# huggingface/tokenizers

Hardware: NVIDIA H100
Metric: encode_batch input throughput (higher is better)
Workload: dtype u8

## Files before the change

### tokenizers_b200/csrc/engine.cu

```cuda
#include <cuda_runtime.h>
#include <stdarg.h>
#include <stdio.h>
#include <stdlib.h>
#include <string.h>

#include <algorithm>
#include <atomic>
#include <condition_variable>
#include <memory>
#include <mutex>
#include <string>
#include <vector>

#include "../../include/b2t.h"
#include "added_kernels.cuh"
#include "dense_kernels.cuh"
#include "host_tables.h"
#include "long_kernels.cuh"
#include "model_kernels.cuh"
#include "norm_kernels.cuh"
#include "prefix_kernels.cuh"
#include "pretok_kernels.cuh"

using namespace b2t;
// ... 269 lines not shown
    long long v = atoll(cb);
    if (v >= 1024 && v < (1ll << 31)) e->chunk_bytes = (size_t)v;
  }
  int rc = B2T_OK;
  if ((rc = upload(e->d_cls, ht.cls_packed)) || (rc = upload(e->d_byte_to_id, ht.byte_to_id)) || (rc = upload(e->d_merge, ht.merge_tbl)) ||
      (rc = upload(e->d_word, ht.word_tbl)) || (rc = upload(e->d_pool, ht.word_pool)) || (rc = upload(e->d_edge, ht.edge_tbl)) ||
      (rc = upload(e->d_tok2, ht.tok2_bits)) || (rc = upload(e->d_tri, ht.tri_bits)))
    return rc;
  if (cfg->bert_normalizer & B2T_NORM_BERT) {
    NormHost nh;
    build_bert_norm((cfg->bert_normalizer & B2T_NORM_CLEAN_TEXT) != 0, (cfg->bert_normalizer & B2T_NORM_CHINESE_CHARS) != 0,
                    (cfg->bert_normalizer & B2T_NORM_STRIP_ACCENTS) != 0, (cfg->bert_normalizer & B2T_NORM_LOWERCASE) != 0, &nh);
    if (!nh.ok) return fail(B2T_ERR_UNSUPPORTED, "BertNormalizer table: an image exceeds three bytes per input byte");
    if ((rc = upload(e->d_nt_blk, nh.blk)) || (rc = upload(e->d_nt_ent, nh.ent)) || (rc = upload(e->d_nt_pool, nh.pool)) || (rc = upload(e->d_nt_ascii, nh.ascii)))
      return rc;
    e->nt.blk = e->d_nt_blk.as<uint16_t>(); e->nt.ent = e->d_nt_ent.as<uint32_t>(); e->nt.pool = e->d_nt_pool.as<uint8_t>(); e->nt.ascii = e->d_nt_ascii.as<uint8_t>();
    e->norm_on = 1;
  }
  memset(&e->dt, 0, sizeof(e->dt));
  e->dt.byte_to_id = e->d_byte_to_id.as<uint32_t>();
  e->dt.merge_tbl = e->d_merge.as<uint4>();
  e->dt.merge_mask = ht.merge_tbl.empty() ? 0 : (uint32_t)ht.merge_tbl.size() - 1;
  e->dt.word_tbl = e->d_word.as<uint4>();
  e->dt.word_mask = ht.word_tbl.empty() ? 0 : (uint32_t)ht.word_tbl.size() - 1;
  e->dt.word_pool = e->d_pool.as<uint8_t>();
  e->dt.ignore_merges = cfg->ignore_merges ? 1 : 0;
  e->dt.monotone = ht.monotone ? 1 : 0;
  e->dt.tok2_bits = e->d_tok2.as<uint32_t>(); e->dt.tri_bits = e->d_tri.as<uint32_t>();
  e->monotone = e->dt.monotone;
  e->dt.edge_tbl = e->d_edge.as<uint4>();
  e->dt.edge_mask = ht.edge_tbl.empty() ? 0 : (uint32_t)ht.edge_tbl.size() - 1;
  e->dt.unk_id = ht.unk_id;
  e->dt.max_chars = ht.max_chars;
  cudaFuncSetAttribute(model_tile_kernel<MODEL_BPE>, cudaFuncAttributePreferredSharedMemoryCarveout, 86);
  cudaFuncSetAttribute(model_tile_kernel<MODEL_WORDPIECE>, cudaFuncAttributePreferredSharedMemoryCarveout, 86);
  if (cfg->model == B2T_MODEL_BPE) {
    if ((rc = upload(e->d_trim_vocab, vocab_trim_counts(cfg->n_vocab, cfg->vocab_bytes, cfg->vocab_off, cfg->vocab_ids)))) return rc;
    e->trim_ready = 1;
  }
  cudaError_t se = cudaStreamCreateWithFlags(&e->own_stream, cudaStreamNonBlocking);
  if (se != cudaSuccess) return fail(B2T_ERR_CUDA, "cudaStreamCreate failed: %s", cudaGetErrorString(se));
  *out = e.release();
  return B2T_OK;
}

extern "C" void b2t_engine_destroy(b2t_engine* e) {
  if (!e) return;
  cudaSetDevice(e->device);
  cudaDeviceSynchronize();
  delete e;
}

struct ctl_block {
  uint32_t max_row;
  uint32_t err;
  unsigned long long total;
  LongCtl lc;
  uint32_t added_used;
  uint32_t max_all;
  unsigned long long rows;
  uint32_t stride_m;
  uint32_t pad;
};

static int ensure_long_pool(Workspace& ws, unsigned long long bytes) {
  if (bytes <= ws.pool_cap) return B2T_OK;
  unsigned long long cap = bytes + bytes / 4 + 4096;
  int rc;
// ... 358 lines not shown
    case PT_GPT2: launch_pretok<PT_GPT2>(e, d_bytes, n, ws, st, added); break;
    case PT_LLAMA3: launch_pretok<PT_LLAMA3>(e, d_bytes, n, ws, st, added); break;
    case PT_WHITESPACE: launch_pretok<PT_WHITESPACE>(e, d_bytes, n, ws, st, added); break;
    case PT_BERT: launch_pretok<PT_BERT>(e, d_bytes, n, ws, st, added); break;
    default: launch_pretok<PT_NOREGEX>(e, d_bytes, n, ws, st, added); break;
  }
  rec(e, st, "pretok_scan"); e->last_launches++;
  const int64_t n_scan_blocks = (n_pages + SCAN_BLOCK - 1) / SCAN_BLOCK;
  page_scan_block_kernel<<<(unsigned)n_scan_blocks, SCAN_BLOCK, 0, st>>>(ws.page_sum.as<uint64_t>(), ws.page_carry.as<uint64_t>(),
                                                                      ws.block_sum.as<uint64_t>(), n_pages);
  page_scan_top_kernel<<<1, SCAN_BLOCK, 0, st>>>(ws.block_sum.as<uint64_t>(), ws.block_carry.as<uint64_t>(), n_scan_blocks);
  rec(e, st, "page_scan"); e->last_launches += 2;
  return B2T_OK;
}

static void long_pretokens(b2t_engine* e, Workspace& ws, const Batch& b, cudaStream_t st) {
  const uint8_t* d_bytes = b.bytes; const int64_t n = b.n;
  const int64_t n_pages = n / PAGE + 1;
  ctl_block* ctl = ws.ctl.as<ctl_block>();
  LongPool pool;
  pool.id = ws.lp_id.as<uint32_t>(); pool.val = ws.lp_val.as<uint64_t>(); pool.len = ws.lp_len.as<uint32_t>(); pool.plen = ws.lp_plen.as<uint32_t>();
  pool.aux = ws.lp_aux.as<uint32_t>(); pool.out = ws.lp_out.as<uint4>(); pool.cap = ws.pool_cap;
  long_find_kernel<0><<<(unsigned)((n_pages + 7) / 8), 256, 0, st>>>(ws.start_bits.as<uint32_t>(), nullptr, nullptr, n, n_pages, &ctl->lc,
                                                                    ws.long_desc1.as<LongDesc>(), nullptr, 0ull);
  soft_cut_kernel<<<(unsigned)(e->sm_count * 4), 256, 0, st>>>(d_bytes, &ctl->lc, ws.long_desc1.as<LongDesc>(), ws.soft_bits.as<uint32_t>(),
                                                             ws.page_soft.as<uint8_t>(), e->dt);
  long_find_kernel<1><<<(unsigned)((n_pages + 7) / 8), 256, 0, st>>>(ws.start_bits.as<uint32_t>(), ws.soft_bits.as<uint32_t>(), ws.page_soft.as<uint8_t>(),
                                                                    n, n_pages, &ctl->lc, ws.long_desc.as<LongDesc>(), ws.page_long.as<int32_t>(), ws.pool_cap);
  rec(e, st, "long_find"); e->last_launches += 3;
  bpe_long_kernel<<<(unsigned)(e->sm_count * 2), LONG_THREADS, 0, st>>>(d_bytes, &ctl->lc, ws.long_desc.as<LongDesc>(), pool, e->dt, e->monotone);
  rec(e, st, "bpe_long"); e->last_launches++;
}

static void model_and_count(b2t_engine* e, Workspace& ws, const Batch& b, uint32_t flags, bool added, cudaStream_t st) {
  const int64_t n_pages = b.n / PAGE + 1;
  ModelParams P;
  P.bytes = b.bytes; P.n = b.n;
  P.start_bits = ws.start_bits.as<uint32_t>(); P.drop_bits = ws.drop_bits.as<uint32_t>(); P.doc_bits = ws.doc_bits.as<uint32_t>();
  P.soft_bits = ws.soft_bits.as<uint32_t>(); P.page_soft = ws.page_soft.as<uint8_t>();
  P.page_carry = ws.page_carry.as<uint64_t>(); P.block_carry = ws.block_carry.as<uint64_t>(); P.page_first_doc = ws.page_first_doc.as<uint32_t>();
  P.doc_off = b.doc_off; P.n_docs = b.n_docs;
  P.flags = ((flags & B2T_WANT_OFFSETS) ? F_OFFSETS : 0u) | ((flags & B2T_WANT_WORD_IDS) ? F_WORD_IDS : 0u) |
            (((flags & B2T_OFFSETS_BYTES) || ws.norm_active) ? F_BYTE_OFFSETS : 0u);
  P.ids = ws.tmp_ids.as<uint32_t>(); P.offsets = ws.tmp_offsets.as<uint32_t>(); P.word_ids = ws.tmp_word_ids.as<uint32_t>();
  P.row_ptr = ws.row_ptr_local.as<uint64_t>();
  P.tile_count = ws.tile_count.as<uint32_t>(); P.tile_first = ws.tile_first.as<uint32_t>();
  ctl_block* ctl = ws.ctl.as<ctl_block>();
  P.err_flag = &ctl->err;
  P.n_tiles = n_pages;
  P.page_long = ws.page_long.as<int32_t>(); P.long_desc = ws.long_desc.as<LongDesc>(); P.long_out = ws.lp_out.as<uint4>();
  P.wcache = ws.wcache.as<uint4>(); P.wcache_mask = WCACHE_SLOTS - 1; P.wcache_on = e->wcache_on;
  P.prefix_bits = b.prefix_bits;
  P.added_bits = added ? ws.added_bits.as<uint32_t>() : nullptr; P.added_head = ws.added_head.as<uint32_t>(); P.added_pool = ws.added_pool.as<uint2>();
  P.flag_added = (flags & B2T_FLAG_ADDED_IDS) ? 1u : 0u;
  P.t = e->dt;
  if (e->model == B2T_MODEL_BPE) model_tile_kernel<MODEL_BPE><<<(unsigned)n_pages, MODEL_THREADS, 0, st>>>(P);
  else model_tile_kernel<MODEL_WORDPIECE><<<(unsigned)n_pages, MODEL_THREADS, 0, st>>>(P);
  rec(e, st, e->model == B2T_MODEL_BPE ? "bpe_tile" : "wordpiece_tile"); e->last_launches++;
  const int64_t n_tblk = (n_pages + TSCAN - 1) / TSCAN;
  tile_scan_block_kernel<<<(unsigned)n_tblk, TSCAN, 0, st>>>(ws.tile_count.as<uint32_t>(), ws.tile_lexcl.as<unsigned long long>(),
                                                           ws.tile_bsum.as<unsigned long long>(), n_pages);
  tile_scan_top_kernel<<<1, TSCAN, 0, st>>>(ws.tile_bsum.as<unsigned long long>(), n_tblk, &ctl->total);
  e->last_launches += 2;
}

static int finish_tail(b2t_engine* e, Workspace& ws, cudaStream_t st) {
  const DenseReq* dq = ws.req.dq;
  const bool finish = ws.req.until == RUN_RESULT;
  const uint32_t n_docs = ws.batch.n_docs;
  int rc;
  if (finish && (rc = finish_device(e, ws, ws.ids.as<uint32_t>(), ws.offsets.as<uint32_t>(), ws.word_ids.as<uint32_t>(), ws.row_ptr.as<uint64_t>(), 0ull, st)))
    return rc;
  rec(e, st, "scan_compact");
  if (dq && finish) {
    ctl_block* ctl = ws.ctl.as<ctl_block>();
    const uint32_t n_rows = n_docs / dq->docs_per_row;
    const PairDenseSpec& P = dq->P;
    if (n_rows && dq->pairs())
      pair_len_max_kernel<<<(n_rows + 255) / 256, 256, 0, st>>>(ws.row_ptr.as<uint64_t>(), n_rows, P.budget, P.strategy, P.n_pre + P.n_mid + P.n_post,
                                                              &ctl->max_row, &ctl->err);
    else if (n_rows)
      row_len_max_kernel<<<(n_rows + 255) / 256, 256, 0, st>>>(ws.row_ptr.as<uint64_t>(), n_rows, dq->S.keep_max, dq->S.n_pre + dq->S.n_post, &ctl->max_row);
    e->last_launches++;
    if (dq->overflow) {
      const uint32_t budget = dq->pairs() ? P.budget : dq->S.keep_max, n_special = dq->pairs() ? P.n_pre + P.n_mid + P.n_post : dq->S.n_pre + dq->S.n_post;
      const int64_t n_blk = ((int64_t)n_rows + TSCAN - 1) / TSCAN;
      if ((rc = ws.row_count.ensure((size_t)n_rows * 4 + 16)) || (rc = ws.row_lexcl.ensure((size_t)n_rows * 8 + 16)) ||
          (rc = ws.row_bsum.ensure((size_t)n_blk * 8 + 16)))
        return rc;
      if (n_rows) {
        dense_count_kernel<<<(n_rows + 255) / 256, 256, 0, st>>>(ws.row_ptr.as<uint64_t>(), n_rows, dq->pairs() ? 1u : 0u, budget, dq->pairs() ? P.strategy : 0u, dq->stride,
                                                               n_special, ws.row_count.as<uint32_t>(), &ctl->max_all, &ctl->err, &ctl->stride_m);
        tile_scan_block_kernel<<<(unsigned)n_blk, TSCAN, 0, st>>>(ws.row_count.as<uint32_t>(), ws.row_lexcl.as<unsigned long long>(),
                                                                 ws.row_bsum.as<unsigned long long>(), n_rows);
        tile_scan_top_kernel<<<1, TSCAN, 0, st>>>(ws.row_bsum.as<unsigned long long>(), n_blk, &ctl->rows);
        e->last_launches += 3;
      }
      rec(e, st, "dense_count");
    } else {
      if (!dq->batch_longest && (rc = launch_dense(e, ws, n_rows, n_rows, *dq, st))) return rc;
      rec(e, st, dq->pairs() ? "dense_pair_rows" : "dense_rows");
    }
  }
  CU(cudaMemcpyAsync(ws.h_ctl.p, ws.ctl.p, sizeof(ctl_block), cudaMemcpyDeviceToHost, st));
  return B2T_OK;
}

static int run_device_pipeline(b2t_engine* e, Workspace& ws, cudaStream_t st) {
  const Request& q = ws.req;
  if (q.n + (int64_t)q.n_docs >= (1ll << 31)) return fail(B2T_ERR_TOO_LARGE, "batch of %lld bytes exceeds the per-call limit of 2^31-1; split it", (long long)q.n);
  Batch& b = ws.batch;
  b = Batch{q.bytes, q.n, q.doc_off, q.n_docs, nullptr};
  e->last_launches = 0;
  const bool model_pass = q.until != RUN_PRETOK;
  int rc;
  if ((rc = repack_prefix(e, ws, b, st)) || (rc = normalize(e, ws, b, q.flags, st)) || (rc = size_buffers(e, ws, b, q.flags, model_pass, st)))
    return rc;
  const bool added = e->has_added && !(q.flags & B2T_NO_ADDED_TOKENS) && b.n > 0 && b.n_docs > 0;
  if ((rc = scan(e, ws, b, added, st))) return rc;
  if (model_pass) {
    if (e->model == B2T_MODEL_BPE) long_pretokens(e, ws, b, st);
    model_and_count(e, ws, b, q.flags, added, st);
    if ((rc = finish_tail(e, ws, st))) return rc;
  }
  CU(cudaGetLastError());
  return B2T_OK;
}

static int trim_ambiguous() {
  return fail(B2T_ERR_UNSUPPORTED, "offset trimming: an added token with both lstrip and rstrip absorbed whitespace, and its offsets do not tell "
              "on which side; trim_offsets is not available for this batch");
}

static int meta_check(b2t_engine* e, Workspace& ws, const DenseReq& dq, cudaStream_t st) {
  if (!dq.trim || !e->has_added || !e->added_both) return B2T_OK;
  ctl_block* h = ws.h_ctl.as<ctl_block>();
  CU(cudaMemcpyAsync(&h->err, &ws.ctl.as<ctl_block>()->err, 4, cudaMemcpyDeviceToHost, st));
  CU(cudaStreamSynchronize(st));
  if (h->err & ERR_INTERNAL) return fail(B2T_ERR_CUDA, "internal error: a marked added-token id without an added token");
  return (h->err & ERR_TRIM_AMBIGUOUS) ? trim_ambiguous() : B2T_OK;
}

static int check_run(b2t_engine* e, Workspace& ws, cudaStream_t st, bool* reran = nullptr) {
  for (int attempt = 0;; ++attempt) {
    const ctl_block* c = ws.h_ctl.as<ctl_block>();
    if (c->err & ERR_ADDED_UNSUPPORTED)
      return fail(B2T_ERR_UNSUPPORTED, "added-token extraction: a span over %d bytes, more spans than one per 16 input bytes, or overlapping spans; "
                  "pass B2T_NO_ADDED_TOKENS and split on the host", ADDED_MAX_SPAN);
    if ((c->err | c->lc.err) & ERR_INTERNAL) return fail(B2T_ERR_CUDA, "internal error: long pre-token / added-token bookkeeping mismatch");
    if (!(c->lc.err & ERR_POOL_OVERFLOW)) {
      if (c->err & ERR_TRUNCATION) return fail(B2T_ERR_TRUNCATION, "Truncation error: Sequence to truncate too short to respect the provided max_length");
      if (c->err & ERR_STRIDE)
        return fail(B2T_ERR_TRUNCATION, "`stride` must be strictly less than `max_len=%u` (note that `max_len` may be shorter than the max length of the "
                    "original model, as it subtracts the number of special characters", c->stride_m);
      if (c->err & ERR_TRIM_AMBIGUOUS) return trim_ambiguous();
      return B2T_OK;
// ... 575 lines not shown
```

### tokenizers_b200/csrc/model_kernels.cuh

```cuda
#pragma once
#include <cuda_runtime.h>
#include <stdint.h>
#include <type_traits>
#include "b2t_tables.h"
#include "added_kernels.cuh"
#include "long_kernels.cuh"
#include "pretok_logic.cuh"

namespace b2t {

constexpr int TILE = PAGE;
constexpr int MODEL_THREADS = 256;
constexpr int THREAD_PATH_MAX = 32;
enum { MODEL_BPE = 0, MODEL_WORDPIECE = 1 };
enum { F_OFFSETS = 1u, F_WORD_IDS = 2u, F_BYTE_OFFSETS = 4u };
constexpr int MAX_LONG_PER_PAGE = TILE / (LONG_PRETOK_MIN + 1) + 1;

struct ModelParams {
  const uint8_t* bytes; int64_t n;
  const uint32_t* start_bits; const uint32_t* drop_bits; const uint32_t* doc_bits;
  const uint32_t* soft_bits; const uint8_t* page_soft;
  const uint64_t* page_carry; const uint64_t* block_carry; const uint32_t* page_first_doc;
  const uint64_t* doc_off; uint32_t n_docs;
  uint32_t flags;
  uint32_t* ids; uint32_t* offsets; uint32_t* word_ids; uint64_t* row_ptr;
  uint32_t* tile_count; uint32_t* tile_first; uint32_t* err_flag;
  int64_t n_tiles;
  const int32_t* page_long; const LongDesc* long_desc; const uint4* long_out;
  uint4* wcache; uint32_t wcache_mask; int wcache_on;
  const uint32_t* prefix_bits;
  const uint32_t* added_bits; const uint32_t* added_head; const uint2* added_pool; uint32_t flag_added;
  DeviceTables t;
};

__device__ __forceinline__ uint64_t merge_lookup(const DeviceTables& t, uint32_t a, uint32_t b) {
  const uint32_t hf = pair_hash(a, b);
  uint32_t h = hf & t.merge_mask;
  while (true) {
    uint4 e = __ldg(t.merge_tbl + h);
    if (e.x == a && e.y == b) return ((uint64_t)e.z << 32) | e.w;
    if (e.x == EMPTY_KEY) return NO_MERGE;
    h = (h + 1) & t.merge_mask;
  }
}

__device__ __forceinline__ int warp_prefix_words(const uint32_t* bits, uint16_t* pref, int nw, int lane) {
  int c0 = 0, c1 = 0, c2 = 0;
  int i = lane * 3;
  if (i < nw) c0 = __popc(bits[i]);
  if (i + 1 < nw) c1 = __popc(bits[i + 1]);
  if (i + 2 < nw) c2 = __popc(bits[i + 2]);
  int tot = c0 + c1 + c2, inc = tot;
#pragma unroll
  for (int s = 1; s < 32; s <<= 1) {
    int o = __shfl_up_sync(0xFFFFFFFFu, inc, s);
    if (lane >= s) inc += o;
  }
  int ex = inc - tot;
  if (i < nw) pref[i] = (uint16_t)ex;
  if (i + 1 < nw) pref[i + 1] = (uint16_t)(ex + c0);
  if (i + 2 < nw) pref[i + 2] = (uint16_t)(ex + c0 + c1);
  return __shfl_sync(0xFFFFFFFFu, inc, 31);
}

__device__ __forceinline__ uint32_t mask_le(int b) { return b >= 31 ? 0xFFFFFFFFu : ((2u << b) - 1u); }

constexpr int TOK_ID_BITS = 20;
__device__ __forceinline__ uint32_t tok_pack(uint32_t id, int len) { return id | ((uint32_t)len << TOK_ID_BITS); }
__device__ __forceinline__ int tok_len(uint32_t x) { return (int)(x >> TOK_ID_BITS); }
__device__ __forceinline__ uint32_t tok_id(uint32_t x) { return x & ((1u << TOK_ID_BITS) - 1u); }


constexpr int WC_MAX_BYTES = 24, WC_MAX_TOK = 6, WC_PROBES = 4;
constexpr int P4_SPLIT_BYTES = 16;
constexpr int P4_SHORT_G = 8;
#define B2T_WC_READY (1ull << 63)
#define B2T_WC_BUSY (1ull << 62)
#define B2T_WC_FP ((1ull << 62) - 1ull)

struct WordKey {
  uint32_t k[6];
  uint32_t slot;
  unsigned long long fp;
};

__device__ __forceinline__ void wc_make_key(const uint8_t* s_byte, int s, int len, WordKey& key) {
  const uint32_t* w = reinterpret_cast<const uint32_t*>(s_byte) + (s >> 2);
  const uint32_t sh = (uint32_t)(s & 3) * 8u;
  uint32_t a0 = w[0], a1 = w[1], a2 = w[2], a3 = w[3], a4 = w[4], a5 = w[5], a6 = w[6];
  uint32_t k[6] = {__funnelshift_r(a0, a1, sh), __funnelshift_r(a1, a2, sh), __funnelshift_r(a2, a3, sh),
                   __funnelshift_r(a3, a4, sh), __funnelshift_r(a4, a5, sh), __funnelshift_r(a5, a6, sh)};
#pragma unroll
  for (int i = 0; i < 6; ++i) {
    const int v = min(len - 4 * i, 4);
    const uint32_t m = __funnelshift_rc(0xFFFFFFFFu, 0u, (uint32_t)(32 - 8 * v));
    key.k[i] = k[i] & m;
  }
  uint32_t a = key.k[0] ^ (key.k[2] * 0x9E3779B1u) ^ (key.k[4] * 0x85EBCA77u);
// ... 155 lines not shown
          const int q = bp + tok_len(s_tok[bp]);
          s_tok[bp] = tok_pack(nid, nx - bp); s_tok[q] = 0u;
        }
        if (p > bp && p < nx) rk[j] = 0xFFFFFFFFu;
      }
    }
    __syncwarp();
    if (have) {
      const uint32_t newid = tok_id(s_tok[bp]);
#pragma unroll
      for (int j = 0; j < J; ++j) {
        const int p = s + gl + G * j;
        if (p == bp) {
          rk[j] = 0xFFFFFFFFu;
          if (nx < e) { const uint64_t v = merge_lookup(t, newid, tok_id(s_tok[nx])); rk[j] = (uint32_t)(v >> 32); ni[j] = (uint32_t)v; }
        } else if (p == pv) {
          const uint64_t v = merge_lookup(t, tok_id(s_tok[pv]), newid); rk[j] = (uint32_t)(v >> 32); ni[j] = (uint32_t)v;
        }
      }
    }
  }
}


__device__ __forceinline__ int bit_rank_incl(const uint16_t* pref, const uint32_t* bits, int x) {
  return (int)pref[x >> 5] + __popc(bits[x >> 5] & mask_le(x & 31));
}
__device__ __forceinline__ bool bit_at(const uint32_t* bits, int x) { return (bits[x >> 5] >> (x & 31)) & 1u; }

template <int HALO_>
struct PageCommon {
  static constexpr int HALO = HALO_, SPAN = TILE + HALO, NW = SPAN / 32, TW = TILE / 32;
  static_assert(NW <= 96 && SPAN % 16 == 0, "warp_prefix_words handles <= 96 words; tok is 16-byte aligned");
  uint8_t byte[SPAN];
  uint32_t tok[SPAN];
  long long span_doc_start;
  uint32_t startb[NW + 1], keptb[NW + 1], leadb[NW + 1], tokb[NW + 1], dsb[TW + 1], addedb[TW + 1];
  uint16_t apref[NW + 1], spref[NW + 1], lpref[NW + 1], tpref[NW + 1];
  int16_t dlast[TW + 1];
  uint16_t pt[TILE + 2], list[SPAN];
  int tile, npt, elast, is_long, ntok, nmiss;
};
struct BpePage : PageCommon<256> {
  uint16_t mq[TILE / THREAD_PATH_MAX + 2], lk[MAX_LONG_PER_PAGE + 1];
  int nmiss_hi, nmq, anysoft, nl, lcum[MAX_LONG_PER_PAGE + 2];
  unsigned long long loff[MAX_LONG_PER_PAGE + 1];
};
struct WpPage : PageCommon<416> {
  long long long_end;
  int next, long_chars;
};
template <int MODEL> using PageState = std::conditional_t<MODEL == MODEL_BPE, BpePage, WpPage>;

__device__ __forceinline__ int long_tokens_before(const BpePage& sh, int x) {
  int c = 0;
  for (int a = 0; a < sh.nl; ++a) if ((int)sh.pt[sh.lk[a]] < x) c = sh.lcum[a + 1];
  return c;
}
__device__ __forceinline__ int long_tokens_before(const WpPage&, int) { return 0; }

__device__ __forceinline__ bool is_piece(const BpePage& sh, int64_t base, int64_t n, int s, int e) {
  if (!sh.anysoft) return false;
  const bool real_e = base + e >= n || (e < BpePage::SPAN && bit_at(sh.keptb, e));
  return !(bit_at(sh.keptb, s) && real_e);
}

template <class S>
__device__ __forceinline__ bool added_at(const ModelParams& P, const S& sh, int s) { return P.added_bits != nullptr && bit_at(sh.addedb, s); }
__device__ __forceinline__ uint32_t added_id(const ModelParams& P, int64_t t, int s) {
  for (uint32_t i = __ldg(P.added_head + t); i != ADDED_NIL;) {
    const uint2 v = __ldg(P.added_pool + i);
    if ((int)(v.x & (uint32_t)(PAGE - 1)) == s) return v.x >> 11;
    i = v.y;
  }
  atomicOr(P.err_flag, ERR_INTERNAL);
  return 0u;
}

__device__ __forceinline__ void warp_enqueue(uint16_t* q, int* len, bool take, int k, bool back) {
  const int lane = threadIdx.x & 31;
  const unsigned m = __ballot_sync(0xFFFFFFFFu, take);
  int b = 0;
  if (lane == 0 && m) b = atomicAdd(len, __popc(m));
  b = __shfl_sync(0xFFFFFFFFu, b, 0) + __popc(m & ((1u << lane) - 1u));
  if (take) q[back ? -b : b] = (uint16_t)k;
}

__device__ __forceinline__ bool whole_word_gate(const ModelParams& P, const uint8_t* s_byte, uint32_t* s_tok, int s, int e, bool ask, int leader) {
  if (!P.t.ignore_merges) return false;
  const int whole = ask && vocab_whole_word(P.t, s_byte, s, e - s, s_tok) ? 1 : 0;
  return __shfl_sync(0xFFFFFFFFu, whole, leader) != 0;
}

__device__ __forceinline__ int64_t char_boundary(const ModelParams& P, int64_t g, int step) {
  while ((step < 0 ? g > 0 : g < P.n) && (__ldg(P.bytes + g) & 0xC0u) == 0x80u) g += step;
  return g;
}

struct DocOrigin { int64_t ds; int cb; uint32_t wid; };
template <class S>
__device__ __forceinline__ DocOrigin doc_origin(const ModelParams& P, const S& sh, int64_t base, int x) {
  const int xx = x < TILE ? x : TILE - 1;
  const uint32_t m = sh.dsb[xx >> 5] & mask_le(xx & 31);
  const int D = m ? (xx & ~31) + 31 - __clz((int)m) : (int)sh.dlast[xx >> 5];
  int2 carry = make_int2(0, 0);
  if (D < 0) {
    const uint64_t c = __ldg(P.page_carry + sh.tile);
    const uint64_t bc = (c >> 31) & 1ull ? 0ull : __ldg(P.block_carry + (sh.tile >> 10));
    carry = make_int2((int)(((uint32_t)c & 0x7FFFFFFFu) + (uint32_t)bc), (int)((uint32_t)(c >> 32) + (uint32_t)(bc >> 32)));
  }
  DocOrigin o;
  o.ds = D >= 0 ? base + D : sh.span_doc_start;
  o.cb = D >= 0 ? bit_rank_incl(sh.lpref, sh.leadb, D) - 1 : -carry.x;
  const int wb = D >= 0 ? bit_rank_incl(sh.spref, sh.keptb, D) - (int)bit_at(sh.keptb, D) : -carry.y;
  o.wid = (uint32_t)(bit_rank_incl(sh.spref, sh.keptb, x) - 1 - wb);
  return o;
}

__device__ __forceinline__ void place_token(const ModelParams& P, const DocOrigin& o, unsigned long long out,
                                            int c0, int c1, int64_t g0, int64_t g1) {
  if (P.flags & F_OFFSETS) {
    const bool byte_off = P.flags & F_BYTE_OFFSETS;
    uint32_t o0, o1;
    if (!byte_off) {
      o0 = (uint32_t)(c0 - o.cb); o1 = (uint32_t)(c1 - o.cb);
    } else {
      o0 = (uint32_t)(char_boundary(P, g0, -1) - o.ds); o1 = (uint32_t)(char_boundary(P, g1, 1) - o.ds);
    }
    if (P.prefix_bits && ((__ldg(P.prefix_bits + (o.ds >> 5)) >> (o.ds & 31)) & 1u)) {
      if (o1 == 1u && byte_off) o1 = (uint32_t)(char_boundary(P, o.ds + 2, 1) - o.ds);
      o0 = o0 ? o0 - 1u : 0u;
      o1 = o1 > 2u ? o1 - 1u : 1u;
    }
    reinterpret_cast<uint2*>(P.offsets)[out] = make_uint2(o0, o1);
  }
  if (P.flags & F_WORD_IDS) P.word_ids[out] = o.wid;
}

template <class S>
__device__ __forceinline__ void emit_token(const ModelParams& P, const S& sh, int64_t base, unsigned long long out,
                                           uint32_t id, int ts, int c1, int64_t g1) {
  P.ids[out] = (P.flag_added && ts < TILE && added_at(P, sh, ts)) ? (id | 0x80000000u) : id;
  place_token(P, doc_origin(P, sh, base, ts), out, bit_rank_incl(sh.lpref, sh.leadb, ts) - 1, c1, base + ts, g1);
}

struct PageSpan { int first, eproc, pproc; bool is_long, long_kept; };
template <int MODEL, class S>
__device__ __forceinline__ PageSpan page_span(const S& sh) {
  const int Pn = sh.npt;
  PageSpan r;
  r.is_long = sh.is_long && Pn > 0;
  const bool wp_long = MODEL == MODEL_WORDPIECE && r.is_long;
  r.first = Pn ? (int)sh.pt[0] : sh.elast;
  r.eproc = Pn ? (wp_long ? (int)sh.pt[Pn - 1] : sh.elast) : 0;
  r.pproc = wp_long ? Pn - 1 : Pn;
  r.long_kept = wp_long && bit_at(sh.keptb, sh.pt[Pn - 1]);
  return r;
}

template <int MODEL, class S>
__device__ __forceinline__ void stage_page(const ModelParams& P, S& sh, int64_t t, int64_t base) {
  constexpr int SPAN = S::SPAN, NW = S::NW, TW = S::TW;
  const int tid = threadIdx.x, lane = tid & 31, warp = tid >> 5;
  const int64_t n = P.n, n_chunks = n / CHUNK + 1;
  for (int i = tid; i < SPAN / 16; i += MODEL_THREADS) {
    int64_t g = base + (int64_t)i * 16;
    uint4 v = make_uint4(0, 0, 0, 0);
    if (g + 16 <= n) v = __ldg(reinterpret_cast<const uint4*>(P.bytes + g));
    else if (g < n) {
      uint32_t w[4] = {0, 0, 0, 0};
      for (int k = 0; k < 16 && g + k < n; ++k) w[k >> 2] |= (uint32_t)__ldg(P.bytes + g + k) << (8 * (k & 3));
      v = make_uint4(w[0], w[1], w[2], w[3]);
    }
    reinterpret_cast<uint4*>(sh.byte)[i] = v;
  }
  for (int w = tid; w <= NW; w += MODEL_THREADS) {
// ... 55 lines not shown
          while (e < 0) {
            int64_t w = gw + lane;
            uint32_t b = (w < n_chunks) ? __ldg(P.start_bits + w) : 0u;
            uint32_t any = __ballot_sync(0xFFFFFFFFu, b != 0u);
            if (any) {
              int l = __ffs((int)any) - 1;
              uint32_t bb = __shfl_sync(0xFFFFFFFFu, b, l);
              e = (gw + l) * 32 + (__ffs((int)bb) - 1);
            } else if (gw + 32 >= n_chunks) e = n;
            gw += 32;
          }
          if (lane == 0) sh.long_end = e < n ? e : n;
        }
      }
    } else if (found > lim) found = (int)lim;
    if (lane == 0) { sh.elast = found; sh.is_long = is_long; }
  } else if (warp == 4) {
    uint32_t b0 = sh.dsb[2 * lane], b1 = sh.dsb[2 * lane + 1];
    int last0 = b0 ? (2 * lane) * 32 + 31 - __clz((int)b0) : -1;
    int last1 = b1 ? (2 * lane + 1) * 32 + 31 - __clz((int)b1) : -1;
    int mx = max(last0, last1), inc = mx;
#pragma unroll
    for (int s = 1; s < 32; s <<= 1) {
      int o = __shfl_up_sync(0xFFFFFFFFu, inc, s);
      if (lane >= s) inc = max(inc, o);
    }
    int before = __shfl_up_sync(0xFFFFFFFFu, inc, 1);
    if (lane == 0) before = -1;
    sh.dlast[2 * lane] = (int16_t)before; sh.dlast[2 * lane + 1] = (int16_t)max(before, last0);
    if (lane == 31) sh.dlast[TW] = (int16_t)inc;
  } else if (warp == 5 && lane == 0) {
    uint32_t fd = __ldg(P.page_first_doc + t);
    sh.span_doc_start = fd > 0 ? (long long)__ldg(P.doc_off + fd - 1) : 0;
  }
  __syncthreads();
  if (tid < S::TW) {
    uint32_t bits = sh.startb[tid];
    int idx = sh.apref[tid];
    while (bits) { sh.pt[idx++] = (uint16_t)(tid * 32 + __ffs((int)bits) - 1); bits &= bits - 1u; }
  }
  if (tid == 0) sh.pt[sh.npt] = (uint16_t)sh.elast;
}

__device__ __forceinline__ void collect_long_pretokens(const ModelParams& P, BpePage& sh, int64_t t, int64_t base) {
  const int tid = threadIdx.x, Pn = sh.npt;
  int any_long = 0;
  for (int k = tid; k < Pn; k += MODEL_THREADS)
    if ((int)sh.pt[k + 1] - (int)sh.pt[k] > LONG_PRETOK_MIN) { int i = atomicAdd(&sh.nl, 1); if (i < MAX_LONG_PER_PAGE) sh.lk[i] = (uint16_t)k; any_long = 1; }
  if (!__syncthreads_or(any_long)) return;
  if (tid == 0) {
    int nl = sh.nl;
    if (nl > MAX_LONG_PER_PAGE) { nl = MAX_LONG_PER_PAGE; atomicOr(P.err_flag, ERR_INTERNAL); }
    for (int a = 1; a < nl; ++a) { uint16_t v = sh.lk[a]; int b = a - 1; while (b >= 0 && sh.lk[b] > v) { sh.lk[b + 1] = sh.lk[b]; --b; } sh.lk[b + 1] = v; }
    const int32_t slot0 = nl ? __ldg(P.page_long + t) : 0;
    if (nl && slot0 < 0) { atomicOr(P.err_flag, ERR_INTERNAL); nl = 0; }
    int cum = 0;
    for (int a = 0; a < nl; ++a) {
      const LongDesc d = P.long_desc[slot0 + a];
      if (d.start != base + sh.pt[sh.lk[a]]) atomicOr(P.err_flag, ERR_INTERNAL);
      sh.lcum[a] = cum; sh.loff[a] = d.pool_off;
      cum += (d.pool_off == ~0ull) ? 0 : (int)d.ntok;
    }
    sh.lcum[nl] = cum;
    sh.nl = nl;
  }
  __syncthreads();
  for (int a = 0; a < sh.nl; ++a) {
    const int ls = sh.pt[sh.lk[a]], le = min((int)sh.pt[sh.lk[a] + 1], BpePage::SPAN);
    for (int pos = ls + tid; pos < le; pos += MODEL_THREADS) sh.tok[pos] = 0u;
  }
  __syncthreads();
}
// ... 87 lines not shown
        }
        if (best_end < 0) { bad = true; break; }
        sh.tok[start] = tok_pack(best_id, best_end - start);
        start = best_end;
      }
    }
    if (bad) {
      for (int p = s; p < e; ++p) sh.tok[p] = 0u;
      sh.tok[s] = tok_pack(P.t.unk_id, len);
    }
    wc_publish(P, sh.byte, sh.tok, s, e, false);
  }
  if (sp.is_long) {
    const int64_t ls = base + sh.pt[sh.npt - 1], le = sh.long_end;
    int cnt = 0;
    for (int64_t p = ls + tid; p < le; p += MODEL_THREADS) cnt += ((__ldg(P.bytes + p) & 0xC0u) != 0x80u);
#pragma unroll
    for (int sft = 16; sft >= 1; sft >>= 1) cnt += __shfl_xor_sync(0xFFFFFFFFu, cnt, sft);
    if (lane == 0) atomicAdd(&sh.long_chars, cnt);
  }
}

template <int MODEL, class S>
__device__ __forceinline__ void count_tokens(const ModelParams& P, S& sh, int64_t t, int64_t base) {
  const int tid = threadIdx.x, lane = tid & 31;
  const PageSpan sp = page_span<MODEL>(sh);
  for (int row = tid >> 5; row < S::NW; row += MODEL_THREADS / 32) {
    const int pos = row * 32 + lane;
    const uint32_t tb = __ballot_sync(0xFFFFFFFFu, pos >= sp.first && pos < sp.eproc && tok_len(sh.tok[pos]) != 0);
    if (lane == 0) sh.tokb[row] = tb;
  }
  __syncthreads();
  if (tid < 32) {
    const int tot = warp_prefix_words(sh.tokb, sh.tpref, S::NW, lane);
    if (lane == 0) sh.ntok = tot;
  }
  __syncthreads();
  for (int row = tid >> 5; row < S::NW; row += MODEL_THREADS / 32) {
    const uint32_t tb = sh.tokb[row];
    if ((tb >> lane) & 1u) sh.list[sh.tpref[row] + __popc(tb & ((1u << lane) - 1u))] = (uint16_t)(row * 32 + lane);
  }
  if (tid == 0) {
    P.tile_count[t] = (uint32_t)(sh.ntok + long_tokens_before(sh, TILE) + (sp.long_kept ? 1 : 0));
    P.tile_first[t] = (uint32_t)(base + sp.first);
  }
}

template <int MODEL, class S>
__device__ __forceinline__ void emit_tokens(const ModelParams& P, const S& sh, int64_t base) {
  const PageSpan sp = page_span<MODEL>(sh);
  const unsigned long long excl = (unsigned long long)(base + sp.first);
  const int n_normal = sh.ntok;
  for (int j = threadIdx.x; j < n_normal; j += MODEL_THREADS) {
    const int pos = sh.list[j];
    const uint32_t tk = sh.tok[pos];
    const int e = pos + tok_len(tk);
    emit_token(P, sh, base, excl + (unsigned long long)(j + long_tokens_before(sh, pos)), tok_id(tk), pos,
               bit_rank_incl(sh.lpref, sh.leadb, e - 1), base + e);
  }
  if constexpr (MODEL == MODEL_BPE) {
    for (int a = 0; a < sh.nl; ++a) {
      const int ls = sh.pt[sh.lk[a]];
      const int ntl = sh.lcum[a + 1] - sh.lcum[a];
      if (ntl == 0) continue;
      const uint4* __restrict__ lo = P.long_out + sh.loff[a];
      const int nb = ls == 0 ? 0 : bit_rank_incl(sh.tpref, sh.tokb, ls - 1);
      const unsigned long long obase = excl + (unsigned long long)(nb + sh.lcum[a]);
      const int X = bit_rank_incl(sh.lpref, sh.leadb, ls) - 1;
      const DocOrigin o = doc_origin(P, sh, base, ls);
      for (int k = threadIdx.x; k < ntl; k += MODEL_THREADS) {
        const uint4 r = lo[k];
        P.ids[obase + k] = r.x;
        place_token(P, o, obase + k, X + (int)r.z, X + (int)r.w, base + ls + (k ? (int64_t)lo[k - 1].y : 0), base + ls + (int64_t)r.y);
      }
    }
  } else if (sp.long_kept && threadIdx.x == 0) {
    const int ls = sh.pt[sh.npt - 1];
    emit_token(P, sh, base, excl + (unsigned long long)sh.ntok, P.t.unk_id, ls,
               bit_rank_incl(sh.lpref, sh.leadb, ls) - 1 + sh.long_chars, sh.long_end);
  }
}

template <class S>
__device__ __forceinline__ void write_row_ptr(const ModelParams& P, const S& sh, int64_t t, int64_t base) {
  const uint32_t fd = __ldg(P.page_first_doc + t);
  for (uint64_t d = (uint64_t)fd + threadIdx.x; d <= P.n_docs; d += MODEL_THREADS) {
    const int64_t pos = (int64_t)__ldg(P.doc_off + d) - base;
    if (pos >= TILE) break;
    const int before = pos == 0 ? 0 : bit_rank_incl(sh.tpref, sh.tokb, (int)pos - 1);
    P.row_ptr[d] = (unsigned long long)(before + long_tokens_before(sh, (int)pos));
  }
}

constexpr int MODEL_MINBLOCKS = 8;
template <int MODEL>
__global__ void __launch_bounds__(MODEL_THREADS, MODEL_MINBLOCKS) model_tile_kernel(const ModelParams P) {
  __shared__ __align__(16) PageState<MODEL> sh;
  const int tid = threadIdx.x;
  if (tid == 0) {
    sh.tile = (int)blockIdx.x;
    sh.nmiss = 0;
    if constexpr (MODEL == MODEL_BPE) { sh.nmiss_hi = 0; sh.nmq = 0; sh.anysoft = 0; sh.nl = 0; sh.lcum[0] = 0; }
    else { sh.next = 0; sh.long_chars = 0; }
  }
  __syncthreads();
  const int64_t t = sh.tile;
  if (t >= P.n_tiles) return;
  const int64_t base = t * TILE;

  stage_page<MODEL>(P, sh, t, base);
  __syncthreads();
  if constexpr (MODEL == MODEL_BPE) {
    collect_long_pretokens(P, sh, t, base);
    resolve_bpe(P, sh, t, base);
  } else {
    resolve_wordpiece(P, sh, t, base);
  }
  __syncthreads();
  count_tokens<MODEL>(P, sh, t, base);
  __syncthreads();
  emit_tokens<MODEL>(P, sh, base);
  write_row_ptr(P, sh, t, base);
}


constexpr int TSCAN = 1024;

__device__ __forceinline__ unsigned long long block_excl_scan(unsigned long long v, unsigned long long* s_w) {
  const int lane = threadIdx.x & 31, warp = threadIdx.x >> 5;
  auto warp_incl_scan = [lane](unsigned long long x) {
#pragma unroll
    for (int s = 1; s < 32; s <<= 1) { unsigned long long o = __shfl_up_sync(0xFFFFFFFFu, x, s); if (lane >= s) x += o; }
    return x;
  };
  const unsigned long long inc = warp_incl_scan(v);
  if (lane == 31) s_w[warp] = inc;
  __syncthreads();
  if (warp == 0) { const unsigned long long w = s_w[lane]; s_w[lane] = warp_incl_scan(w) - w; }
  __syncthreads();
  return s_w[warp] + inc - v;
}

__global__ void __launch_bounds__(TSCAN) tile_scan_block_kernel(const uint32_t* __restrict__ cnt, unsigned long long* __restrict__ local_excl,
                                                                unsigned long long* __restrict__ block_sum, int64_t n_tiles) {
  __shared__ unsigned long long s_w[32];
  const int64_t i = (int64_t)blockIdx.x * TSCAN + threadIdx.x;
  const unsigned long long v = i < n_tiles ? (unsigned long long)cnt[i] : 0ull;
  const unsigned long long ex = block_excl_scan(v, s_w);
  if (i < n_tiles) local_excl[i] = ex;
  if (threadIdx.x == TSCAN - 1) block_sum[blockIdx.x] = ex + v;
}

__global__ void __launch_bounds__(TSCAN) tile_scan_top_kernel(unsigned long long* __restrict__ block_sum, int64_t n_blocks, unsigned long long* __restrict__ total) {
  __shared__ unsigned long long s_w[32];
  __shared__ unsigned long long s_run;
// ... 60 lines not shown
```

Before: 55.58.

## Specialize page model kernel per output layout and precompute token prefix ranks

Templates the page tokenization kernel on an output-layout bitmask (offsets, word ids, byte offsets, prefix, added ids), so unused output paths compile away, and dispatches through a host table of kernel instantiations. It also drops the compacted token list: emission iterates token bitmask rows directly, and per-word token prefixes now fold in long-pretoken counts, replacing the per-token long_tokens_before loops. Per-word doc carry values are precomputed once in shared memory, so doc_origin no longer reloads page/block carry from global memory. The cost is many more kernel instantiations (binary size, compile time), somewhat more shared memory per block from the new int arrays, and a new error path for unsupported layouts.

```diff
diff --git a/tokenizers_b200/csrc/engine.cu b/tokenizers_b200/csrc/engine.cu
--- a/tokenizers_b200/csrc/engine.cu
+++ b/tokenizers_b200/csrc/engine.cu
@@ -325,8 +325,10 @@
   e->dt.edge_mask = ht.edge_tbl.empty() ? 0 : (uint32_t)ht.edge_tbl.size() - 1;
   e->dt.unk_id = ht.unk_id;
   e->dt.max_chars = ht.max_chars;
-  cudaFuncSetAttribute(model_tile_kernel<MODEL_BPE>, cudaFuncAttributePreferredSharedMemoryCarveout, 86);
-  cudaFuncSetAttribute(model_tile_kernel<MODEL_WORDPIECE>, cudaFuncAttributePreferredSharedMemoryCarveout, 86);
+  for (int i = 0; i < N_MODEL_LAYOUTS; ++i) {
+    cudaFuncSetAttribute(model_kernel<MODEL_BPE>(i), cudaFuncAttributePreferredSharedMemoryCarveout, 86);
+    cudaFuncSetAttribute(model_kernel<MODEL_WORDPIECE>(i), cudaFuncAttributePreferredSharedMemoryCarveout, 86);
+  }
   if (cfg->model == B2T_MODEL_BPE) {
     if ((rc = upload(e->d_trim_vocab, vocab_trim_counts(cfg->n_vocab, cfg->vocab_bytes, cfg->vocab_off, cfg->vocab_ids)))) return rc;
     e->trim_ready = 1;
@@ -751,16 +753,20 @@
   rec(e, st, "bpe_long"); e->last_launches++;
 }
 
-static void model_and_count(b2t_engine* e, Workspace& ws, const Batch& b, uint32_t flags, bool added, cudaStream_t st) {
+static int model_and_count(b2t_engine* e, Workspace& ws, const Batch& b, uint32_t flags, bool added, cudaStream_t st) {
   const int64_t n_pages = b.n / PAGE + 1;
+  const bool offs = flags & B2T_WANT_OFFSETS;
+  const unsigned lay = (offs ? L_OFFSETS : 0u) | ((flags & B2T_WANT_WORD_IDS) ? L_WORD_IDS : 0u) |
+                       (offs && ((flags & B2T_OFFSETS_BYTES) || ws.norm_active) ? L_BYTE_OFFSETS : 0u) |
+                       (offs && b.prefix_bits ? L_PREFIX : 0u) | (added && (flags & B2T_FLAG_ADDED_IDS) ? L_ADDED_IDS : 0u);
+  const int li = model_layout_index(lay);
+  if (li < 0) return fail(B2T_ERR_INVALID, "no page kernel for output layout %u", lay);
   ModelParams P;
   P.bytes = b.bytes; P.n = b.n;
   P.start_bits = ws.start_bits.as<uint32_t>(); P.drop_bits = ws.drop_bits.as<uint32_t>(); P.doc_bits = ws.doc_bits.as<uint32_t>();
   P.soft_bits = ws.soft_bits.as<uint32_t>(); P.page_soft = ws.page_soft.as<uint8_t>();
   P.page_carry = ws.page_carry.as<uint64_t>(); P.block_carry = ws.block_carry.as<uint64_t>(); P.page_first_doc = ws.page_first_doc.as<uint32_t>();
   P.doc_off = b.doc_off; P.n_docs = b.n_docs;
-  P.flags = ((flags & B2T_WANT_OFFSETS) ? F_OFFSETS : 0u) | ((flags & B2T_WANT_WORD_IDS) ? F_WORD_IDS : 0u) |
-            (((flags & B2T_OFFSETS_BYTES) || ws.norm_active) ? F_BYTE_OFFSETS : 0u);
   P.ids = ws.tmp_ids.as<uint32_t>(); P.offsets = ws.tmp_offsets.as<uint32_t>(); P.word_ids = ws.tmp_word_ids.as<uint32_t>();
   P.row_ptr = ws.row_ptr_local.as<uint64_t>();
   P.tile_count = ws.tile_count.as<uint32_t>(); P.tile_first = ws.tile_first.as<uint32_t>();
@@ -771,16 +777,16 @@
   P.wcache = ws.wcache.as<uint4>(); P.wcache_mask = WCACHE_SLOTS - 1; P.wcache_on = e->wcache_on;
   P.prefix_bits = b.prefix_bits;
   P.added_bits = added ? ws.added_bits.as<uint32_t>() : nullptr; P.added_head = ws.added_head.as<uint32_t>(); P.added_pool = ws.added_pool.as<uint2>();
-  P.flag_added = (flags & B2T_FLAG_ADDED_IDS) ? 1u : 0u;
   P.t = e->dt;
-  if (e->model == B2T_MODEL_BPE) model_tile_kernel<MODEL_BPE><<<(unsigned)n_pages, MODEL_THREADS, 0, st>>>(P);
-  else model_tile_kernel<MODEL_WORDPIECE><<<(unsigned)n_pages, MODEL_THREADS, 0, st>>>(P);
+  const ModelKernel k = e->model == B2T_MODEL_BPE ? model_kernel<MODEL_BPE>(li) : model_kernel<MODEL_WORDPIECE>(li);
+  k<<<(unsigned)n_pages, MODEL_THREADS, 0, st>>>(P);
   rec(e, st, e->model == B2T_MODEL_BPE ? "bpe_tile" : "wordpiece_tile"); e->last_launches++;
   const int64_t n_tblk = (n_pages + TSCAN - 1) / TSCAN;
   tile_scan_block_kernel<<<(unsigned)n_tblk, TSCAN, 0, st>>>(ws.tile_count.as<uint32_t>(), ws.tile_lexcl.as<unsigned long long>(),
                                                            ws.tile_bsum.as<unsigned long long>(), n_pages);
   tile_scan_top_kernel<<<1, TSCAN, 0, st>>>(ws.tile_bsum.as<unsigned long long>(), n_tblk, &ctl->total);
   e->last_launches += 2;
+  return B2T_OK;
 }
 
 static int finish_tail(b2t_engine* e, Workspace& ws, cudaStream_t st) {
@@ -839,8 +845,7 @@
   if ((rc = scan(e, ws, b, added, st))) return rc;
   if (model_pass) {
     if (e->model == B2T_MODEL_BPE) long_pretokens(e, ws, b, st);
-    model_and_count(e, ws, b, q.flags, added, st);
-    if ((rc = finish_tail(e, ws, st))) return rc;
+    if ((rc = model_and_count(e, ws, b, q.flags, added, st)) || (rc = finish_tail(e, ws, st))) return rc;
   }
   CU(cudaGetLastError());
   return B2T_OK;
diff --git a/tokenizers_b200/csrc/model_kernels.cuh b/tokenizers_b200/csrc/model_kernels.cuh
--- a/tokenizers_b200/csrc/model_kernels.cuh
+++ b/tokenizers_b200/csrc/model_kernels.cuh
@@ -2,6 +2,7 @@
 #include <cuda_runtime.h>
 #include <stdint.h>
 #include <type_traits>
+#include <utility>
 #include "b2t_tables.h"
 #include "added_kernels.cuh"
 #include "long_kernels.cuh"
@@ -13,8 +14,16 @@
 constexpr int MODEL_THREADS = 256;
 constexpr int THREAD_PATH_MAX = 32;
 enum { MODEL_BPE = 0, MODEL_WORDPIECE = 1 };
-enum { F_OFFSETS = 1u, F_WORD_IDS = 2u, F_BYTE_OFFSETS = 4u };
 constexpr int MAX_LONG_PER_PAGE = TILE / (LONG_PRETOK_MIN + 1) + 1;
+
+enum : unsigned { L_OFFSETS = 1u, L_WORD_IDS = 2u, L_BYTE_OFFSETS = 4u, L_PREFIX = 8u, L_ADDED_IDS = 16u };
+constexpr unsigned MODEL_LAYOUTS[] = {0u, 1u, 5u, 9u, 13u, 2u, 3u, 7u, 11u, 15u, 16u, 17u, 21u, 25u, 29u, 18u, 19u, 23u, 27u, 31u};
+constexpr int N_MODEL_LAYOUTS = (int)(sizeof(MODEL_LAYOUTS) / sizeof(MODEL_LAYOUTS[0]));
+constexpr int model_layout_index(unsigned lay) {
+  for (int i = 0; i < N_MODEL_LAYOUTS; ++i)
+    if (MODEL_LAYOUTS[i] == lay) return i;
+  return -1;
+}
 
 struct ModelParams {
   const uint8_t* bytes; int64_t n;
@@ -22,14 +31,13 @@
   const uint32_t* soft_bits; const uint8_t* page_soft;
   const uint64_t* page_carry; const uint64_t* block_carry; const uint32_t* page_first_doc;
   const uint64_t* doc_off; uint32_t n_docs;
-  uint32_t flags;
   uint32_t* ids; uint32_t* offsets; uint32_t* word_ids; uint64_t* row_ptr;
   uint32_t* tile_count; uint32_t* tile_first; uint32_t* err_flag;
   int64_t n_tiles;
   const int32_t* page_long; const LongDesc* long_desc; const uint4* long_out;
   uint4* wcache; uint32_t wcache_mask; int wcache_on;
   const uint32_t* prefix_bits;
-  const uint32_t* added_bits; const uint32_t* added_head; const uint2* added_pool; uint32_t flag_added;
+  const uint32_t* added_bits; const uint32_t* added_head; const uint2* added_pool;
   DeviceTables t;
 };
 
@@ -44,7 +52,8 @@
   }
 }
 
-__device__ __forceinline__ int warp_prefix_words(const uint32_t* bits, uint16_t* pref, int nw, int lane) {
+template <class T>
+__device__ __forceinline__ int warp_prefix_words(const uint32_t* bits, T* pref, int nw, int lane) {
   int c0 = 0, c1 = 0, c2 = 0;
   int i = lane * 3;
   if (i < nw) c0 = __popc(bits[i]);
@@ -57,13 +66,14 @@
     if (lane >= s) inc += o;
   }
   int ex = inc - tot;
-  if (i < nw) pref[i] = (uint16_t)ex;
-  if (i + 1 < nw) pref[i + 1] = (uint16_t)(ex + c0);
-  if (i + 2 < nw) pref[i + 2] = (uint16_t)(ex + c0 + c1);
+  if (i < nw) pref[i] = (T)ex;
+  if (i + 1 < nw) pref[i + 1] = (T)(ex + c0);
+  if (i + 2 < nw) pref[i + 2] = (T)(ex + c0 + c1);
   return __shfl_sync(0xFFFFFFFFu, inc, 31);
 }
 
 __device__ __forceinline__ uint32_t mask_le(int b) { return b >= 31 ? 0xFFFFFFFFu : ((2u << b) - 1u); }
+__device__ __forceinline__ uint32_t mask_lt(int b) { return (1u << b) - 1u; }
 
 constexpr int TOK_ID_BITS = 20;
 __device__ __forceinline__ uint32_t tok_pack(uint32_t id, int len) { return id | ((uint32_t)len << TOK_ID_BITS); }
@@ -285,14 +295,16 @@
 struct PageCommon {
   static constexpr int HALO = HALO_, SPAN = TILE + HALO, NW = SPAN / 32, TW = TILE / 32;
   static_assert(NW <= 96 && SPAN % 16 == 0, "warp_prefix_words handles <= 96 words; tok is 16-byte aligned");
+  static_assert(2 * TW <= MODEL_THREADS, "stage_page: one thread per word of the page for pt, one for dcb / dwb");
   uint8_t byte[SPAN];
   uint32_t tok[SPAN];
   long long span_doc_start;
   uint32_t startb[NW + 1], keptb[NW + 1], leadb[NW + 1], tokb[NW + 1], dsb[TW + 1], addedb[TW + 1];
-  uint16_t apref[NW + 1], spref[NW + 1], lpref[NW + 1], tpref[NW + 1];
+  int tpref[NW + 1], dcb[TW], dwb[TW];
+  uint16_t apref[NW + 1], spref[NW + 1], lpref[NW + 1];
   int16_t dlast[TW + 1];
   uint16_t pt[TILE + 2], list[SPAN];
-  int tile, npt, elast, is_long, ntok, nmiss;
+  int tile, npt, elast, is_long, ntok, nmiss, carry_c, carry_w;
 };
 struct BpePage : PageCommon<256> {
   uint16_t mq[TILE / THREAD_PATH_MAX + 2], lk[MAX_LONG_PER_PAGE + 1];
@@ -305,13 +317,6 @@
 };
 template <int MODEL> using PageState = std::conditional_t<MODEL == MODEL_BPE, BpePage, WpPage>;
 
-__device__ __forceinline__ int long_tokens_before(const BpePage& sh, int x) {
-  int c = 0;
-  for (int a = 0; a < sh.nl; ++a) if ((int)sh.pt[sh.lk[a]] < x) c = sh.lcum[a + 1];
-  return c;
-}
-__device__ __forceinline__ int long_tokens_before(const WpPage&, int) { return 0; }
-
 __device__ __forceinline__ bool is_piece(const BpePage& sh, int64_t base, int64_t n, int s, int e) {
   if (!sh.anysoft) return false;
   const bool real_e = base + e >= n || (e < BpePage::SPAN && bit_at(sh.keptb, e));
@@ -351,50 +356,55 @@
 }
 
 struct DocOrigin { int64_t ds; int cb; uint32_t wid; };
-template <class S>
-__device__ __forceinline__ DocOrigin doc_origin(const ModelParams& P, const S& sh, int64_t base, int x) {
-  const int xx = x < TILE ? x : TILE - 1;
-  const uint32_t m = sh.dsb[xx >> 5] & mask_le(xx & 31);
-  const int D = m ? (xx & ~31) + 31 - __clz((int)m) : (int)sh.dlast[xx >> 5];
-  int2 carry = make_int2(0, 0);
-  if (D < 0) {
-    const uint64_t c = __ldg(P.page_carry + sh.tile);
-    const uint64_t bc = (c >> 31) & 1ull ? 0ull : __ldg(P.block_carry + (sh.tile >> 10));
-    carry = make_int2((int)(((uint32_t)c & 0x7FFFFFFFu) + (uint32_t)bc), (int)((uint32_t)(c >> 32) + (uint32_t)(bc >> 32)));
-  }
+template <unsigned LAY, class S>
+__device__ __forceinline__ DocOrigin doc_origin(const S& sh, int64_t base, int x) {
+  const int xx = x < TILE ? x : TILE - 1, w = xx >> 5;
+  const uint32_t m = sh.dsb[w] & mask_le(xx & 31);
   DocOrigin o;
-  o.ds = D >= 0 ? base + D : sh.span_doc_start;
-  o.cb = D >= 0 ? bit_rank_incl(sh.lpref, sh.leadb, D) - 1 : -carry.x;
-  const int wb = D >= 0 ? bit_rank_incl(sh.spref, sh.keptb, D) - (int)bit_at(sh.keptb, D) : -carry.y;
-  o.wid = (uint32_t)(bit_rank_incl(sh.spref, sh.keptb, x) - 1 - wb);
+  int wb;
+  if (m) {
+    const int D = (xx & ~31) + 31 - __clz((int)m);
+    o.ds = base + D;
+    o.cb = bit_rank_incl(sh.lpref, sh.leadb, D) - 1;
+    wb = bit_rank_incl(sh.spref, sh.keptb, D) - (int)bit_at(sh.keptb, D);
+  } else {
+    const int D = sh.dlast[w];
+    o.ds = D >= 0 ? base + D : sh.span_doc_start;
+    o.cb = sh.dcb[w];
+    wb = sh.dwb[w];
+  }
+  o.wid = (LAY & L_WORD_IDS) ? (uint32_t)(bit_rank_incl(sh.spref, sh.keptb, x) - 1 - wb) : 0u;
   return o;
 }
 
+template <unsigned LAY>
 __device__ __forceinline__ void place_token(const ModelParams& P, const DocOrigin& o, unsigned long long out,
                                             int c0, int c1, int64_t g0, int64_t g1) {
-  if (P.flags & F_OFFSETS) {
-    const bool byte_off = P.flags & F_BYTE_OFFSETS;
+  if constexpr ((LAY & L_OFFSETS) != 0) {
+    constexpr bool byte_off = (LAY & L_BYTE_OFFSETS) != 0;
     uint32_t o0, o1;
-    if (!byte_off) {
+    if constexpr (!byte_off) {
       o0 = (uint32_t)(c0 - o.cb); o1 = (uint32_t)(c1 - o.cb);
     } else {
       o0 = (uint32_t)(char_boundary(P, g0, -1) - o.ds); o1 = (uint32_t)(char_boundary(P, g1, 1) - o.ds);
     }
-    if (P.prefix_bits && ((__ldg(P.prefix_bits + (o.ds >> 5)) >> (o.ds & 31)) & 1u)) {
-      if (o1 == 1u && byte_off) o1 = (uint32_t)(char_boundary(P, o.ds + 2, 1) - o.ds);
-      o0 = o0 ? o0 - 1u : 0u;
-      o1 = o1 > 2u ? o1 - 1u : 1u;
+    if constexpr ((LAY & L_PREFIX) != 0) {
+      if ((__ldg(P.prefix_bits + (o.ds >> 5)) >> (o.ds & 31)) & 1u) {
+        if (o1 == 1u && byte_off) o1 = (uint32_t)(char_boundary(P, o.ds + 2, 1) - o.ds);
+        o0 = o0 ? o0 - 1u : 0u;
+        o1 = o1 > 2u ? o1 - 1u : 1u;
+      }
     }
     reinterpret_cast<uint2*>(P.offsets)[out] = make_uint2(o0, o1);
   }
-  if (P.flags & F_WORD_IDS) P.word_ids[out] = o.wid;
-}
-
-template <class S>
+  if constexpr ((LAY & L_WORD_IDS) != 0) P.word_ids[out] = o.wid;
+}
+
+template <unsigned LAY, class S>
 __device__ __forceinline__ void emit_token(const ModelParams& P, const S& sh, int64_t base, unsigned long long out,
                                            uint32_t id, int ts, int c1, int64_t g1) {
-  P.ids[out] = (P.flag_added && ts < TILE && added_at(P, sh, ts)) ? (id | 0x80000000u) : id;
-  place_token(P, doc_origin(P, sh, base, ts), out, bit_rank_incl(sh.lpref, sh.leadb, ts) - 1, c1, base + ts, g1);
+  P.ids[out] = ((LAY & L_ADDED_IDS) && ts < TILE && bit_at(sh.addedb, ts)) ? (id | 0x80000000u) : id;
+  place_token<LAY>(P, doc_origin<LAY>(sh, base, ts), out, bit_rank_incl(sh.lpref, sh.leadb, ts) - 1, c1, base + ts, g1);
 }
 
 struct PageSpan { int first, eproc, pproc; bool is_long, long_kept; };
@@ -516,12 +526,20 @@
   } else if (warp == 5 && lane == 0) {
     uint32_t fd = __ldg(P.page_first_doc + t);
     sh.span_doc_start = fd > 0 ? (long long)__ldg(P.doc_off + fd - 1) : 0;
-  }
-  __syncthreads();
-  if (tid < S::TW) {
+    const uint64_t c = __ldg(P.page_carry + t);
+    const uint64_t bc = (c >> 31) & 1ull ? 0ull : __ldg(P.block_carry + (t >> 10));
+    sh.carry_c = (int)(((uint32_t)c & 0x7FFFFFFFu) + (uint32_t)bc);
+    sh.carry_w = (int)((uint32_t)(c >> 32) + (uint32_t)(bc >> 32));
+  }
+  __syncthreads();
+  if (tid < TW) {
     uint32_t bits = sh.startb[tid];
     int idx = sh.apref[tid];
     while (bits) { sh.pt[idx++] = (uint16_t)(tid * 32 + __ffs((int)bits) - 1); bits &= bits - 1u; }
+  } else if (tid < 2 * TW) {
+    const int w = tid - TW, D = sh.dlast[w];
+    sh.dcb[w] = D >= 0 ? bit_rank_incl(sh.lpref, sh.leadb, D) - 1 : -sh.carry_c;
+    sh.dwb[w] = D >= 0 ? bit_rank_incl(sh.spref, sh.keptb, D) - (int)bit_at(sh.keptb, D) : -sh.carry_w;
   }
   if (tid == 0) sh.pt[sh.npt] = (uint16_t)sh.elast;
 }
@@ -675,31 +693,42 @@
   }
   __syncthreads();
   if (tid < 32) {
-    const int tot = warp_prefix_words(sh.tokb, sh.tpref, S::NW, lane);
-    if (lane == 0) sh.ntok = tot;
-  }
-  __syncthreads();
-  for (int row = tid >> 5; row < S::NW; row += MODEL_THREADS / 32) {
-    const uint32_t tb = sh.tokb[row];
-    if ((tb >> lane) & 1u) sh.list[sh.tpref[row] + __popc(tb & ((1u << lane) - 1u))] = (uint16_t)(row * 32 + lane);
-  }
-  if (tid == 0) {
-    P.tile_count[t] = (uint32_t)(sh.ntok + long_tokens_before(sh, TILE) + (sp.long_kept ? 1 : 0));
-    P.tile_first[t] = (uint32_t)(base + sp.first);
-  }
-}
-
-template <int MODEL, class S>
+    int tot = warp_prefix_words(sh.tokb, sh.tpref, S::NW, lane);
+    if constexpr (MODEL == MODEL_BPE) {
+      const int nl = sh.nl;
+      if (nl) {
+        for (int w = lane * 3; w < lane * 3 + 3 && w < S::NW; ++w) {
+          int c = 0;
+          for (int a = 0; a < nl; ++a) if (((int)sh.pt[sh.lk[a]] >> 5) < w) c = sh.lcum[a + 1];
+          sh.tpref[w] += c;
+        }
+        tot += sh.lcum[nl];
+      }
+    }
+    if (lane == 0) {
+      sh.ntok = tot;
+      P.tile_count[t] = (uint32_t)(tot + (sp.long_kept ? 1 : 0));
+      P.tile_first[t] = (uint32_t)(base + sp.first);
+    }
+  }
+}
+
+template <class S>
+__device__ __forceinline__ int tokens_before(const S& sh, int x) { return sh.tpref[x >> 5] + __popc(sh.tokb[x >> 5] & mask_lt(x & 31)); }
+
+template <int MODEL, unsigned LAY, class S>
 __device__ __forceinline__ void emit_tokens(const ModelParams& P, const S& sh, int64_t base) {
   const PageSpan sp = page_span<MODEL>(sh);
   const unsigned long long excl = (unsigned long long)(base + sp.first);
-  const int n_normal = sh.ntok;
-  for (int j = threadIdx.x; j < n_normal; j += MODEL_THREADS) {
-    const int pos = sh.list[j];
+  const int lane = threadIdx.x & 31;
+  for (int row = threadIdx.x >> 5; row < S::NW; row += MODEL_THREADS / 32) {
+    const uint32_t tb = sh.tokb[row];
+    if (!((tb >> lane) & 1u)) continue;
+    const int pos = row * 32 + lane;
     const uint32_t tk = sh.tok[pos];
     const int e = pos + tok_len(tk);
-    emit_token(P, sh, base, excl + (unsigned long long)(j + long_tokens_before(sh, pos)), tok_id(tk), pos,
-               bit_rank_incl(sh.lpref, sh.leadb, e - 1), base + e);
+    emit_token<LAY>(P, sh, base, excl + (unsigned long long)(sh.tpref[row] + __popc(tb & mask_lt(lane))), tok_id(tk), pos,
+                    bit_rank_incl(sh.lpref, sh.leadb, e - 1), base + e);
   }
   if constexpr (MODEL == MODEL_BPE) {
     for (int a = 0; a < sh.nl; ++a) {
@@ -707,20 +736,19 @@
       const int ntl = sh.lcum[a + 1] - sh.lcum[a];
       if (ntl == 0) continue;
       const uint4* __restrict__ lo = P.long_out + sh.loff[a];
-      const int nb = ls == 0 ? 0 : bit_rank_incl(sh.tpref, sh.tokb, ls - 1);
-      const unsigned long long obase = excl + (unsigned long long)(nb + sh.lcum[a]);
+      const unsigned long long obase = excl + (unsigned long long)tokens_before(sh, ls);
       const int X = bit_rank_incl(sh.lpref, sh.leadb, ls) - 1;
-      const DocOrigin o = doc_origin(P, sh, base, ls);
+      const DocOrigin o = doc_origin<LAY>(sh, base, ls);
       for (int k = threadIdx.x; k < ntl; k += MODEL_THREADS) {
         const uint4 r = lo[k];
         P.ids[obase + k] = r.x;
-        place_token(P, o, obase + k, X + (int)r.z, X + (int)r.w, base + ls + (k ? (int64_t)lo[k - 1].y : 0), base + ls + (int64_t)r.y);
+        place_token<LAY>(P, o, obase + k, X + (int)r.z, X + (int)r.w, base + ls + (k ? (int64_t)lo[k - 1].y : 0), base + ls + (int64_t)r.y);
       }
     }
   } else if (sp.long_kept && threadIdx.x == 0) {
     const int ls = sh.pt[sh.npt - 1];
-    emit_token(P, sh, base, excl + (unsigned long long)sh.ntok, P.t.unk_id, ls,
-               bit_rank_incl(sh.lpref, sh.leadb, ls) - 1 + sh.long_chars, sh.long_end);
+    emit_token<LAY>(P, sh, base, excl + (unsigned long long)sh.ntok, P.t.unk_id, ls,
+                    bit_rank_incl(sh.lpref, sh.leadb, ls) - 1 + sh.long_chars, sh.long_end);
   }
 }
 
@@ -730,13 +758,12 @@
   for (uint64_t d = (uint64_t)fd + threadIdx.x; d <= P.n_docs; d += MODEL_THREADS) {
     const int64_t pos = (int64_t)__ldg(P.doc_off + d) - base;
     if (pos >= TILE) break;
-    const int before = pos == 0 ? 0 : bit_rank_incl(sh.tpref, sh.tokb, (int)pos - 1);
-    P.row_ptr[d] = (unsigned long long)(before + long_tokens_before(sh, (int)pos));
+    P.row_ptr[d] = (unsigned long long)tokens_before(sh, (int)pos);
   }
 }
 
 constexpr int MODEL_MINBLOCKS = 8;
-template <int MODEL>
+template <int MODEL, unsigned LAY>
 __global__ void __launch_bounds__(MODEL_THREADS, MODEL_MINBLOCKS) model_tile_kernel(const ModelParams P) {
   __shared__ __align__(16) PageState<MODEL> sh;
   const int tid = threadIdx.x;
@@ -762,8 +789,19 @@
   __syncthreads();
   count_tokens<MODEL>(P, sh, t, base);
   __syncthreads();
-  emit_tokens<MODEL>(P, sh, base);
+  emit_tokens<MODEL, LAY>(P, sh, base);
   write_row_ptr(P, sh, t, base);
+}
+
+using ModelKernel = void (*)(const ModelParams);
+template <int MODEL, int... I>
+struct ModelKernelTable { static constexpr ModelKernel k[sizeof...(I)] = {&model_tile_kernel<MODEL, MODEL_LAYOUTS[I]>...}; };
+template <int MODEL, int... I>
+constexpr ModelKernelTable<MODEL, I...> model_kernel_table(std::integer_sequence<int, I...>) { return {}; }
+template <int MODEL>
+__host__ inline ModelKernel model_kernel(int layout_index) {
+  using T = decltype(model_kernel_table<MODEL>(std::make_integer_sequence<int, N_MODEL_LAYOUTS>{}));
+  return T::k[layout_index];
 }
 
 
```

After: 57.48 (median of 6 runs). 1.03x the previous value.
